# alexaiken/mpas-regent

Measured on NVIDIA B200. Metric: cell_level_updates_per_s, higher is better.
Workload: dtype f64

## Files before the change

mpas_regent_b200/csrc/kernels.cuh:

```cuda
#pragma once
#include "view.h"

#define DI __device__ __forceinline__
#ifndef LB_EDGE
#define LB_EDGE 1
#endif
#ifndef LB_CELLC
#define LB_CELLC 4
#endif
#ifndef LB_CELLC_SPLIT
#define LB_CELLC_SPLIT 5
#endif
#ifndef LB_AC
#define LB_AC 3
#endif
#ifndef KDE_PREFETCH
#define KDE_PREFETCH 1
#endif
#ifndef LB_MISC
#define LB_MISC 1
#endif
#ifndef KDE_MAXREG
#define KDE_MAXREG 56
#endif
// ... 951 lines not shown
  if (m0 && !spec && k0 > 0) s_P[k0] = ac_P(t0, s_rp0[k0 - 1], s_rt0[k0 - 1]);
  __syncthreads();
  if (inx && !spec && k0 == 0) {
    double xv = s_P[0];
#pragma unroll 4
    for (int kk = 1; kk < L; ++kk) { xv = __fma_rn(s_Q[kk], xv, s_P[kk]); s_P[kk] = xv; }
  }
  __syncthreads();
  if (!m0) return;
  const D2 ww_old = S0 ? bc(0.0) : ld2(FLD(wwAvg), ix);
  D2 rw_new, rho_new, rt_new, ww_new;
  if (!spec) {
    const D2 cofrz = ld2(FLD(cofrz), k0), rdzw = ld2(FLD(rdzw), k0);
    const D2 coftz = ld2(FLD(coftz), ix), coftz_p = above(FLD(coftz), ix, k0, L, coftz);
    const D2 rw_oldp = mk(rw_old.y, rw_oldp_y);
    rw_new = mk(s_P[k0], m1 ? s_P[k1] : 0.0);
    const D2 wa = ww_old + 0.5 * (1.0 - epssm) * rw_old;
    const D2 wb = wa + 0.5 * (1.0 + epssm) * rw_new;
    ww_new = mk(k0 > 0 ? wb.x : ww_old.x, wb.y);
    rho_new = rs - cofrz * (rw_oldp - rw_new);
    rt_new = ts - rdzw * (coftz_p * rw_oldp - coftz * rw_new);
  } else {
    const D2 rho_old = S0 ? bc(0.0) : ld2(FLD(rho_pp), ix), rt_old = S0 ? bc(0.0) : ld2(FLD(rtheta_pp), ix);
    rho_new = rho_old + dts * ld2(FLD(tend_rho), ix);
    rt_new = rt_old + dts * ld2(FLD(theta_m), ix);
    rw_new = rw_old + dts * ld2(FLD(w), ix);
    ww_new = ww_old + 0.5 * (1.0 + epssm) * rw_new;
  }
  st2m(FLD(rho_pp), ix, rho_new, m0, m1); st2m(FLD(rtheta_pp), ix, rt_new, m0, m1);
  const bool wr0 = S0 || spec || k0 > 0;
  st2m(FLD(rw_p), ix, rw_new, wr0, m1); st2m(FLD(wwAvg), ix, ww_new, wr0, m1);
}

__global__ void k_acoustic_gather(const View V, double dts) {
  PAIR_THREAD_R()
  XPF_CELL_ROWS();
  if (!m0) return;
  if (V.specZoneMaskCell[x] != 0.0) return;
  const int ME = V.maxEdges, n = V.nEdgesOnCell[x];
  const double inva = V.invAreaCell[x];
  const double* ru_p = FLD(ru_p); const double* tm = FLD(theta_m);
  D2 rs = bc(0), ts = bc(0);
#pragma unroll 2
  for (int i = 0; i < n; ++i) {
    const int e = V.edgesOnCell[x * V.MEP + i];
    const int c1 = V.c1OnCell[x * V.MEP + i], c2 = V.c2OnCell[x * V.MEP + i];
    const D2 flux = V.edgesOnCellSign[x * ME + i] * dts * V.dvOnCell[x * ME + i] * G2(ru_p, e) * inva;
    rs -= flux;
    ts -= flux * 0.5 * (G2(tm, c2) + G2(tm, c1));
  }
  st2m(V.scr_rs, ix, rs, m0, m1); st2m(V.scr_ts, ix, ts, m0, m1);
}

template <bool S0>
__global__ void k_acoustic_u(const View V, double dts, double c2, double gravity) {
  PAIR_THREAD_R()
  if (!m0) return;
  const D2 tru = ld2(FLD(tend_ru), ix);
  if (S0) {
    const D2 r = dts * tru;
    st2m(FLD(ru_p), ix, r, m0, m1); st2m(FLD(ruAvg), ix, r, m0, m1);
    return;
  }
  const int4 cv = V.ecv[x];
  const double* rpp = FLD(rtheta_pp); const double* zz = FLD(zz); const double* ex = FLD(exner); const double* rho = FLD(rho_pp);
  D2 pgrad = ((G2(rpp, cv.y) - G2(rpp, cv.x)) * V.invDcEdge[x]) / (0.5 * (G2(zz, cv.y) + G2(zz, cv.x)));
  pgrad = pgrad * (ld2(FLD(cqu), ix) * 0.5 * c2 * (G2(ex, cv.x) + G2(ex, cv.y)));
  pgrad = pgrad + 0.5 * ld2(FLD(zxu), ix) * gravity * (G2(rho, cv.x) + G2(rho, cv.y));
  const D2 r = ld2(FLD(ru_p), ix) + dts * (tru - (1.0 - V.specZoneMaskEdge[x]) * pgrad);
  st2m(FLD(ru_p), ix, r, m0, m1);
  st2m(FLD(ruAvg), ix, ld2(FLD(ruAvg), ix) + r, m0, m1);
}

template <bool S0>
__global__ void __launch_bounds__(256) k_acoustic_col(const View V, double dts, double epssm, double resm) {
  extern __shared__ double sm[];
  PAIR_THREAD_R()
  const int TS = LP + 2, CB = blockDim.y, ty = threadIdx.y;
  double* s_rs = sm + (size_t)(0 * CB + ty) * TS;
  double* s_ts = sm + (size_t)(1 * CB + ty) * TS;
  double* s_x = sm + (size_t)(2 * CB + ty) * TS;
  double* s_a = sm + (size_t)(3 * CB + ty) * TS;
// ... 209 lines not shown
    double xe = s_P[0];
#pragma unroll 4
    for (int p = 1; p < np; ++p) { xe = __fma_rn(s_Q[p], xe, s_P[p]); s_P[p] = xe; }
  }
  __syncthreads();
  if (!m0) return;
  const D2 ww_old = S0 ? bc(0.0) : ld2(SIN(AF_wwAvg), cl);
  D2 rw_new, rho_new, rt_new, ww_new;
  if (!spec) {
    const double xprev = pr > 0 ? s_P[pr - 1] : 0.0;
    const double x0 = __fma_rn(Q0, xprev, P0);
    rw_new = mk(x0, m1 ? __fma_rn(Q1, x0, P1) : 0.0);
    const D2 wa = ww_old + 0.5 * (1.0 - epssm) * rw_old;
    const D2 wb = wa + 0.5 * (1.0 + epssm) * rw_new;
    ww_new = mk(k0 > 0 ? wb.x : ww_old.x, wb.y);
    rho_new = rs - cofrz * (rw_oldp - rw_new);
    rt_new = ts - rdzw * (coftz_p * rw_oldp - coftz * rw_new);
  } else {
    rho_new = rho_old + dts * ld2(SIN(AF_tend_rho), cl);
    rt_new = rt_old + dts * ld2(SIN(AF_theta_m), cl);
    rw_new = rw_old + dts * ld2(SIN(AF_w), cl);
    ww_new = ww_old + 0.5 * (1.0 + epssm) * rw_new;
  }
  if ((ABL & 4) && rho_new.x != 1.2345e300) return;
  st2m(FLD(rho_pp), ix, rho_new, m0, m1); st2m(FLD(rtheta_pp), ix, rt_new, m0, m1);
  const bool wr0 = S0 || spec || k0 > 0;
  st2m(FLD(rw_p), ix, rw_new, wr0, m1); st2m(FLD(wwAvg), ix, ww_new, wr0, m1);
#undef SIN
}

#ifndef AL_NMOV
#define AL_NMOV 160
#endif
enum { AL_KC = 8, AL_COLS = 32, AL_NOUT = 5 };
DI void mbar_arrive(uint64_t* bar) { asm volatile("mbarrier.arrive.shared::cta.b64 _, [%0];" ::"r"(smem_u32(bar)) : "memory"); }
DI void cp_async_arrive_noinc(uint64_t* bar) { asm volatile("cp.async.mbarrier.arrive.noinc.shared::cta.b64 [%0];" ::"r"(smem_u32(bar)) : "memory"); }
DI void cp_async_16(void* dst, const void* src) { asm volatile("cp.async.cg.shared.global [%0], [%1], 16;" ::"r"(smem_u32(dst)), "l"(src) : "memory"); }
DI void cp_async_8(void* dst, const void* src) { asm volatile("cp.async.ca.shared.global [%0], [%1], 8;" ::"r"(smem_u32(dst)), "l"(src) : "memory"); }
DI int al_off(int c, int p) { return c * AL_KC + (((p ^ (c >> 1)) & 3) << 1); }
struct AcCarry { double rw_prev, rho_prev, rt_prev, zz_m, cofwt_m, rz_m; };
DI void ac_level(int k, bool spec, bool S0, double dts, double epssm, double resm, double cofrz_k, double rdzw_k, double fzm_k, double fzp_k,
                 double tend_rho_k, double theta_m_k, double w_k, double coftz_k, double coftz_p, double cofwz_k, double cofwr_k,
                 double cofwt_k, double a_k, double al_k, double zz_k, double rws_k, double rwv_k, double dsk, double rz_k, double srs_k,
                 double sts_k, double rho_old, double rt_old, double rw_old_k, double rw_old_p, double ww_old, AcCarry& c,
                 double& rho_new, double& rt_new, double& rw_new, double& ww_new) {
  ww_new = ww_old;
  if (!spec) {
    const double rs = rho_old + dts * tend_rho_k + srs_k - cofrz_k * resm * (rw_old_p - rw_old_k);
    const double ts = rt_old + dts * theta_m_k + sts_k - resm * rdzw_k * (coftz_p * rw_old_p - coftz_k * rw_old_k);
    rw_new = rw_old_k;
    if (k > 0) {
      ww_new += 0.5 * (1.0 - epssm) * rw_old_k;
      rw_new += dts * w_k - cofwz_k * ((zz_k * ts - c.zz_m * 0.0) + resm * (zz_k * rt_old - c.zz_m * c.rt_prev))
                - cofwr_k * ((rs + 0.0) + resm * (rho_old + c.rho_prev))
                + cofwt_k * (ts + resm * rt_old)
                + c.cofwt_m * (0.0 + resm * c.rt_prev);
      rw_new -= a_k * c.rw_prev;
      rw_new *= al_k;
      const double r3 = rws_k - rwv_k;
      rw_new += r3 - dts * dsk * (fzm_k * zz_k + fzp_k * c.zz_m) * (fzm_k * rz_k + fzp_k * c.rz_m) * w_k;
      const double r2 = 1.0 + dts * dsk;
      if (r2 != 1.0) rw_new /= r2;
      rw_new -= r3;
      ww_new += 0.5 * (1.0 + epssm) * rw_new;
    }
    rho_new = rs - cofrz_k * (rw_old_p - rw_new);
    rt_new = ts - rdzw_k * (coftz_p * rw_old_p - coftz_k * rw_new);
  } else {
    rho_new = rho_old + dts * tend_rho_k;
    rt_new = rt_old + dts * theta_m_k;
    rw_new = rw_old_k + dts * w_k;
    ww_new = ww_old + 0.5 * (1.0 + epssm) * rw_new;
  }
  c.rw_prev = rw_new; c.rho_prev = rho_new; c.rt_prev = rt_new; c.zz_m = zz_k; c.cofwt_m = cofwt_k; c.rz_m = rz_k;
  (void)S0;
}
template <bool S0>
__global__ void __launch_bounds__(32 + AL_NMOV, 2) k_acoustic_lane(const View V, const AcPtrs F, double dts, double epssm, double resm) {
  extern __shared__ __align__(128) unsigned char smraw[];
  constexpr int NS16 = S0 ? (int)AF_rho_pp : (int)AF_COUNT;
  constexpr int NS8 = S0 ? 1 : 2;
  constexpr int NSTR = NS16 + NS8;
  constexpr int STRIP = AL_COLS * AL_KC;
  double* in = reinterpret_cast<double*>(smraw);
  double* out = in + (size_t)2 * NSTR * STRIP;
  double* s_v = out + (size_t)2 * AL_NOUT * STRIP;
  const int L = V.L, LP = V.LP;
  uint64_t* bars = reinterpret_cast<uint64_t*>(s_v + (size_t)4 * LP);
  uint64_t* full = bars; uint64_t* empty = bars + 2; uint64_t* ofull = bars + 4; uint64_t* oempty = bars + 6;
  const int tid = threadIdx.x, warp = tid >> 5, lane = tid & 31;
  const int nch = (L + AL_KC - 1) / AL_KC;
  const int ntile = (V.xend - V.xoff + AL_COLS - 1) / AL_COLS;
  const int my_tiles = ((int)blockIdx.x < ntile) ? (ntile - 1 - (int)blockIdx.x) / (int)gridDim.x + 1 : 0;
  const int ng = my_tiles * nch;
  if (tid == 0) {
    for (int s = 0; s < 2; ++s) { mbar_init(full + s, AL_NMOV); mbar_init(empty + s, 32); mbar_init(ofull + s, 32); mbar_init(oempty + s, AL_NMOV); }
  }
  for (int i = tid; i < LP; i += blockDim.x) {
    s_v[i] = FLD(cofrz)[i]; s_v[LP + i] = FLD(rdzw)[i]; s_v[2 * LP + i] = FLD(fzm)[i]; s_v[3 * LP + i] = FLD(fzp)[i];
  }
  __syncthreads();
  if (warp == 0) {
    const int c = lane;
    int x = 0; bool on = false, spec = false;
    AcCarry cr; cr.rw_prev = cr.rho_prev = cr.rt_prev = cr.zz_m = cr.cofwt_m = cr.rz_m = 0.0;
    for (int g = 0; g < ng; ++g) {
      const int j = g % nch;
      if (j == 0) {
        x = V.xoff + ((int)blockIdx.x + (g / nch) * (int)gridDim.x) * AL_COLS + c;
        on = x < V.xend;
        spec = on ? (V.specZoneMaskCell[x] != 0.0) : false;
        cr.rw_prev = cr.rho_prev = cr.rt_prev = cr.zz_m = cr.cofwt_m = cr.rz_m = 0.0;
      }
      const int s = g & 1, u = g >> 1;
      mbar_wait(full + s, u & 1);
      if (g >= 2) mbar_wait(oempty + s, (u - 1) & 1);
      const double* __restrict__ si = in + (size_t)s * NSTR * STRIP;
      double* __restrict__ so = out + (size_t)s * AL_NOUT * STRIP;
#pragma unroll
      for (int p = 0; p < AL_KC / 2; ++p) {
        const int k0 = j * AL_KC + 2 * p;
        const int o = al_off(c, p);
#define LDP(f) (*reinterpret_cast<const D2*>(si + (size_t)(f) * STRIP + o))
        const D2 tr = LDP(AF_tend_rho), tm = LDP(AF_theta_m), w2 = LDP(AF_w), cz = LDP(AF_coftz), cwz = LDP(AF_cofwz), cwr = LDP(AF_cofwr),
                 cwt = LDP(AF_cofwt), at = LDP(AF_a_tri), al = LDP(AF_alpha_tri), zz = LDP(AF_zz), rws = LDP(AF_rw_save), rwv = LDP(AF_rw),
                 ds = LDP(AF_dss), rz = LDP(AF_rho_zz), rsh = LDP(AF_rs), tsh = LDP(AF_ts);
        const D2 czn = LDP(NS16);
        D2 rho_o = bc(0.0), rt_o = bc(0.0), rwp = bc(0.0), wwo = bc(0.0), rwpn = bc(0.0);
        if (!S0) { rho_o = LDP(AF_rho_pp); rt_o = LDP(AF_rtheta_pp); rwp = LDP(AF_rw_p); wwo = LDP(AF_wwAvg); rwpn = LDP(NS16 + 1); }
#undef LDP
        D2 rho_n = bc(0.0), rt_n = bc(0.0), rw_n = bc(0.0), ww_n = bc(0.0);
#ifdef AL_ABLATE_SWEEP
        if (false)
#else
        if (on && k0 < L)
#endif
          ac_level(k0, spec, S0, dts, epssm, resm, s_v[k0], s_v[LP + k0], s_v[2 * LP + k0], s_v[3 * LP + k0], tr.x, tm.x, w2.x, cz.x, czn.x,
                   cwz.x, cwr.x, cwt.x, at.x, al.x, zz.x, rws.x, rwv.x, ds.x, rz.x, rsh.x, tsh.x, rho_o.x, rt_o.x, rwp.x, rwpn.x, wwo.x, cr,
                   rho_n.x, rt_n.x, rw_n.x, ww_n.x);
#ifdef AL_ABLATE_SWEEP
        if (false)
#else
        if (on && k0 + 1 < L)
#endif
          ac_level(k0 + 1, spec, S0, dts, epssm, resm, s_v[k0 + 1], s_v[LP + k0 + 1], s_v[2 * LP + k0 + 1], s_v[3 * LP + k0 + 1], tr.y, tm.y, w2.y,
                   cz.y, czn.y, cwz.y, cwr.y, cwt.y, at.y, al.y, zz.y, rws.y, rwv.y, ds.y, rz.y, rsh.y, tsh.y, rho_o.y, rt_o.y, rwp.y, rwpn.y,
                   wwo.y, cr, rho_n.y, rt_n.y, rw_n.y, ww_n.y);
        *reinterpret_cast<D2*>(so + (size_t)0 * STRIP + o) = rho_n;
        *reinterpret_cast<D2*>(so + (size_t)1 * STRIP + o) = rt_n;
        *reinterpret_cast<D2*>(so + (size_t)2 * STRIP + o) = rw_n;
        *reinterpret_cast<D2*>(so + (size_t)3 * STRIP + o) = ww_n;
        *reinterpret_cast<D2*>(so + (size_t)4 * STRIP + o) = rt_o;
      }
      mbar_arrive(empty + s);
      mbar_arrive(ofull + s);
      if (S0 && on && j == nch - 1) { FLD(wwAvg)[(size_t)x * LP + L] = 0; FLD(rw_p)[(size_t)x * LP + L] = 0; }
    }
  } else {
    const int m = tid - 32;
    double* const dst_f[AL_NOUT] = {FLD(rho_pp), FLD(rtheta_pp), FLD(rw_p), FLD(wwAvg), FLD(rtheta_pp_old)};
    const int xl = V.xend - 1;
    for (int g = 0; g <= ng; ++g) {
      if (g < ng) {
        const int s = g & 1, u = g >> 1;
        if (g >= 2) mbar_wait(empty + s, (u - 1) & 1);
        double* si = in + (size_t)s * NSTR * STRIP;
        const int kb = (g % nch) * AL_KC;
        const int x0 = V.xoff + ((int)blockIdx.x + (g / nch) * (int)gridDim.x) * AL_COLS;
        for (int it = m; it < NS16 * (AL_COLS * 4); it += AL_NMOV) {
          const int f = it >> 7, cp = it & 127, c = cp >> 2, p = cp & 3;
          const int xc = min(x0 + c, xl);
          cp_async_16(si + (size_t)f * STRIP + al_off(c, p), F.p[f] + (size_t)xc * LP + kb + 2 * p);
        }
        for (int it = m; it < NS8 * (AL_COLS * 8); it += AL_NMOV) {
          const int f = it >> 8, ck = it & 255, c = ck >> 3, kk = ck & 7;
          const int xc = min(x0 + c, xl);
          const double* src = (f == 0 ? F.p[AF_coftz] : F.p[AF_rw_p]) + (size_t)xc * LP + kb + kk + 1;
          cp_async_8(si + (size_t)(NS16 + f) * STRIP + al_off(c, kk >> 1) + (kk & 1), src);
        }
        cp_async_arrive_noinc(full + s);
      }
      if (g >= 1) {
        const int gg = g - 1, s = gg & 1, u = gg >> 1;
        mbar_wait(ofull + s, u & 1);
        const double* so = out + (size_t)s * AL_NOUT * STRIP;
        const int kb = (gg % nch) * AL_KC;
        const int x0 = V.xoff + ((int)blockIdx.x + (gg / nch) * (int)gridDim.x) * AL_COLS;
        for (int it = m; it < AL_NOUT * (AL_COLS * 4); it += AL_NMOV) {
          const int f = it >> 7, cp = it & 127, c = cp >> 2, p = cp & 3;
          const int x = x0 + c, k0 = kb + 2 * p;
          const D2 v = *reinterpret_cast<const D2*>(so + (size_t)f * STRIP + al_off(c, p));
          if (x < V.xend && k0 < L) st2m(dst_f[f], (size_t)x * LP + k0, v, true, k0 + 1 < L);
        }
        mbar_arrive(oempty + s);
      }
    }
  }
}

__global__ void k_acoustic_flux(const View V, double dts, int small_step) {
  const int k = threadIdx.x;
  const int x = blockIdx.x * blockDim.y + threadIdx.y;
  if (x >= V.nCells) return;
  const int LP = V.LP, L = V.L;
  const size_t ix = (size_t)x * LP + k;
  if (k == L && small_step == 0) { FLD(wwAvg)[ix] = 0; FLD(rw_p)[ix] = 0; }
  if (k >= L) return;
  FLD(rtheta_pp_old)[ix] = (small_step == 0) ? 0.0 : FLD(rtheta_pp)[ix];
  if (V.specZoneMaskCell[x] != 0.0) return;
  const int ME = V.maxEdges, n = V.nEdgesOnCell[x];
  const double* ru_p = FLD(ru_p); const double* tm = FLD(theta_m);
  const double inva = V.invAreaCell[x];
  double rs = 0, ts = 0;
  for (int i = 0; i < n; ++i) {
    const int e = V.edgesOnCell[x * V.MEP + i];
    const int c1 = V.c1OnCell[x * V.MEP + i], c2 = V.c2OnCell[x * V.MEP + i];
    const double flux = V.edgesOnCellSign[x * ME + i] * dts * V.dvOnCell[x * ME + i] * G1(ru_p, e, k) * inva;
    rs -= flux;
    ts -= flux * 0.5 * (G1(tm, c2, k) + G1(tm, c1, k));
  }
  V.scr_rs[ix] = rs; V.scr_ts[ix] = ts;
}
__global__ void k_acoustic_column(const View V, double dts, int small_step, double epssm, double resm) {
  const int c = blockIdx.x * blockDim.x + threadIdx.x;
  if (c >= V.nCells) return;
  const int L = V.L, LP = V.LP;
  const size_t b = (size_t)c * LP;
  const bool S0 = small_step == 0;
// ... 453 lines not shown
```

mpas_regent_b200/csrc/mpas_b200.cu:

```cuda
#include <cuda_runtime.h>
#include <dlfcn.h>

#include <algorithm>
#include <cmath>
#include <cstdio>
#include <cstddef>
#include <cstdlib>
#include <cstring>
#include <map>
#include <mutex>
#include <numeric>
#include <string>
#include <vector>

#include "kernels.cuh"
#ifdef MPASB200_LAB
#include "kernels_tiles.cuh"
#endif
#include "kernels_init.cuh"
#include "kernels_jw.cuh"
#ifdef MPASB200_LAB
#include "kernels_staged.cuh"
#include "kernels_lab.cuh"
#endif
// ... 384 lines not shown
Range range_of(const mpasb200_t* h, int ent, int n) {
  if (!h->rangeSet[ent]) return Range{0, n, n, true};
  const int b = std::min(h->rangeB[ent], n), e = std::min(h->rangeE[ent], n);
  return Range{b, e, std::max(0, e - b), b == 0 && e == n};
}
View ranged(const mpasb200_t* h, const Range& r) { View v = h->V; v.xoff = r.b; v.xend = r.e; return v; }
int t_smlstep(mpasb200_t* h) { LAUNCH(k_smlstep, h->nCells, 0, h->V, h->c.nRelaxZone); return post_launch(h); }
int t_acoustic(mpasb200_t* h, double dts, int small_step) {
  const double epssm = h->c.config_epssm;
  const double resm = (1.0 - epssm) / (1.0 + epssm);
  const Range rc_ = range_of(h, MPASB200_CELL, h->nCells), re_ = range_of(h, MPASB200_EDGE, h->nEdges);
  const View Vc = ranged(h, rc_), Ve = ranged(h, re_);
  const size_t sm_gather = staged_bytes(h, 12, 0);
  if (h->c.physics_mode == MPASB200_PHYSICS_CORRECTED) {
    const double rcv = h->c.rgas / (h->c.cp - h->c.rgas), c2 = h->c.cp * rcv;
    if (small_step == 0) LAUNCH(k_acoustic_u<true>, re_.n, 0, Ve, dts, c2, h->c.gravity);
    else LAUNCH(k_acoustic_u<false>, re_.n, 0, Ve, dts, c2, h->c.gravity);
    if (staged_on(h, GS_AC_GATHER, sm_gather)) LAUNCH_STAGED(k_acoustic_gather_s<6>, rc_.n, sm_gather, Vc, dts);
    else LAUNCH(k_acoustic_gather, rc_.n, 0, Vc, dts);
    if (small_step == 0) LAUNCH(k_acoustic_col<true>, rc_.n, tile_bytes(h, 6), Vc, dts, epssm, resm);
    else LAUNCH(k_acoustic_col<false>, rc_.n, tile_bytes(h, 6), Vc, dts, epssm, resm);
    return post_launch(h);
  }
  {
    const size_t smem_lane = ((size_t)2 * (AF_COUNT + 2) * AL_COLS * AL_KC + (size_t)2 * AL_NOUT * AL_COLS * AL_KC + (size_t)4 * h->LP) * sizeof(double) + 64;
    if (!h->c.acoustic_exact && h->c.acoustic_tma == 3 && smem_lane <= (size_t)h->max_smem_optin) {
      if (rc_.n == 0) return 0;
      const View& V = Vc;
      AcPtrs F;
#define AF(n) F.p[AF_##n] = V.f[MPASB200_F_##n]
      AF(tend_rho); AF(theta_m); AF(w); AF(coftz); AF(cofwz); AF(cofwr); AF(cofwt); AF(a_tri); AF(alpha_tri); AF(zz); AF(rw_save); AF(rw);
      AF(dss); AF(rho_zz); AF(rho_pp); AF(rtheta_pp); AF(rw_p); AF(wwAvg);
#undef AF
      F.p[AF_rs] = V.scr_rs; F.p[AF_ts] = V.scr_ts;
      LAUNCH(k_acoustic_gather, rc_.n, 0, Vc, dts);
      static bool attr_ = false;
      if (!attr_) {
        cudaFuncSetAttribute(k_acoustic_lane<true>, cudaFuncAttributeMaxDynamicSharedMemorySize, h->max_smem_optin);
        cudaFuncSetAttribute(k_acoustic_lane<false>, cudaFuncAttributeMaxDynamicSharedMemorySize, h->max_smem_optin);
        attr_ = true;
      }
      const size_t smem0 = ((size_t)2 * ((int)AF_rho_pp + 1) * AL_COLS * AL_KC + (size_t)2 * AL_NOUT * AL_COLS * AL_KC + (size_t)4 * h->LP) * sizeof(double) + 64;
      const int tiles = (rc_.n + AL_COLS - 1) / AL_COLS;
      const dim3 grid(std::min(tiles, 2 * h->num_sms)), block(32 + AL_NMOV);
      {
        KTimer kt_(h, small_step == 0 ? "k_acoustic_lane<true>" : "k_acoustic_lane<false>");
        if (small_step == 0) k_acoustic_lane<true><<<grid, block, smem0, h->stream>>>(V, F, dts, epssm, resm);
        else k_acoustic_lane<false><<<grid, block, smem_lane, h->stream>>>(V, F, dts, epssm, resm);
      }
      h->launches++;
      return post_launch(h);
    }
  }
  const bool tma_fits = ((size_t)AF_COUNT * h->LP + (size_t)4 * (h->LP + 2)) * sizeof(double) + 16 <= 48 * 1024 && h->LP / 2 <= 128;
  if (!h->c.acoustic_exact && h->c.acoustic_tma && h->nCells > 0 && tma_fits) {
    if (rc_.n == 0) return 0;
    const View& V = Vc;
    AcPtrs F;
#define AF(n) F.p[AF_##n] = V.f[MPASB200_F_##n]
    AF(tend_rho); AF(theta_m); AF(w); AF(coftz); AF(cofwz); AF(cofwr); AF(cofwt); AF(a_tri); AF(alpha_tri); AF(zz); AF(rw_save); AF(rw);
    AF(dss); AF(rho_zz); AF(rho_pp); AF(rtheta_pp); AF(rw_p); AF(wwAvg);
#undef AF
    F.p[AF_rs] = V.scr_rs; F.p[AF_ts] = V.scr_ts;
    const int split = h->c.acoustic_tma == 2;
    if (split) {
      if (staged_on(h, GS_AC_GATHER, sm_gather)) LAUNCH_STAGED(k_acoustic_gather_s<6>, rc_.n, sm_gather, Vc, dts);
      else LAUNCH(k_acoustic_gather, rc_.n, 0, Vc, dts);
    }
    const int T = h->LP / 2, NF = small_step == 0 ? (int)AF_rho_pp : (int)AF_COUNT;
    int C = 4;
    auto smem_for = [&](int c) { return ((size_t)NF * c * h->LP + (size_t)4 * c * (h->LP + 2)) * sizeof(double) + 16; };
    while (C > 1 && (smem_for(C) > 48 * 1024 || C * T > 128)) C /= 2;
    const size_t smem = smem_for(C);
    dim3 block(T, C), grid((rc_.n + C - 1) / C);
// ... 354 lines not shown
  c->config_horiz_mixing = MPASB200_MIX_2D_SMAGORINSKY;
  c->nRelaxZone = 5; c->number_of_sub_steps = 2; c->config_dynamics_split_steps = 1;
  c->index_policy = MPASB200_INDEX_CORRECTED; c->rkarg_policy = MPASB200_RKARG_SUBSTEP_TRUNC;
  c->sfc_renumber = 1; c->device = -1; c->use_graph = 0; c->acoustic_exact = 0; c->acoustic_tma = 3;
  c->physics_mode = MPASB200_PHYSICS_LITERAL;
  c->gather_stage = 0;
  c->config_scalar_advection = 0; c->config_coef_3rd_order = 0.25;
  c->edge_tiles = 0; c->kernel_forms = 0; c->reserved0 = 0;
}

const char* mpasb200_last_error(const mpasb200_t* h) { return h ? h->err.c_str() : g_create_error.c_str(); }

int mpasb200_create(const MpasDims* dims, const MpasConfig* cfg, mpasb200_t** out) {
  if (!dims || !cfg || !out) return fail(nullptr, MPASB200_EINVAL, "null argument");
  if (dims->nCells < 0 || dims->nEdges < 0 || dims->nVertices < 0 || dims->nVertLevels < 3)
    return fail(nullptr, MPASB200_EINVAL, "bad dimensions (nVertLevels must be >= 3)");
  if (dims->maxEdges < 1 || dims->maxEdges > 16 || dims->nAdvCells < 1 || dims->vertexDegree != 3)
    return fail(nullptr, MPASB200_EINVAL, "unsupported maxEdges / nAdvCells / vertexDegree");
  int ndev = 0;
  cudaError_t e = cudaGetDeviceCount(&ndev);
  if (e != cudaSuccess || ndev == 0)
    return fail(nullptr, MPASB200_ENODEVICE, std::string("no CUDA device (") + cudaGetErrorString(e) + "); libmpas_b200 has no host path");
  mpasb200_t* h = new mpasb200();
  h->d = *dims; h->c = *cfg;
  if (cfg->device >= 0) h->device = cfg->device; else cudaGetDevice(&h->device);
  if ((e = cudaSetDevice(h->device)) != cudaSuccess) { g_create_error = std::string("cudaSetDevice: ") + cudaGetErrorString(e); delete h; return MPASB200_ECUDA; }
  h->nCells = dims->nCells; h->nEdges = dims->nEdges; h->nVertices = dims->nVertices;
  h->L = dims->nVertLevels; h->L1 = h->L + 1; h->LP = (h->L1 + 3) / 4 * 4;
  { const int T = h->LP / 2; int g = T, b = 32; while (b) { int t = g % b; g = b; b = t; } h->CPB = 32 / g; while (h->CPB * T < 128) h->CPB *= 2;
    while (h->CPB * T > 256 && h->CPB > 1) h->CPB /= 2; }
  if (h->LP / 2 * h->CPB > 256) { g_create_error = "nVertLevels too large for one block per column group"; delete h; return MPASB200_EINVAL; }
  cudaDeviceGetAttribute(&h->num_sms, cudaDevAttrMultiProcessorCount, h->device);
  cudaDeviceGetAttribute(&h->max_smem_optin, cudaDevAttrMaxSharedMemoryPerBlockOptin, h->device);
  cudaStreamCreateWithFlags(&h->own_stream, cudaStreamNonBlocking);
  h->stream = h->own_stream;
  cudaEventCreate(&h->ev0); cudaEventCreate(&h->ev1);
  View& V = h->V;
  std::memset(&V, 0, sizeof(V));
  V.nCells = h->nCells; V.nEdges = h->nEdges; V.nVertices = h->nVertices; V.L = h->L; V.LP = h->LP;
  V.xoff = 0; V.xend = 0;
  V.maxEdges = dims->maxEdges; V.maxEdges2 = dims->maxEdges2; V.vertexDegree = dims->vertexDegree; V.nAdv = dims->nAdvCells;
  V.cellSlot = (size_t)(h->nCells + 1) * h->LP;
  size_t total = 0;
  std::vector<size_t> off(MPASB200_F_COUNT);
  for (int id = 0; id < MPASB200_F_COUNT; ++id) {
    size_t n = (kFields[id].entity == MPASB200_VERTICAL) ? (size_t)h->LP
                                                         : (size_t)(entity_count(h, kFields[id].entity) + 1) * h->LP * kFields[id].slots;
    n = (n + 15) / 16 * 16;
    off[id] = total; total += n;
  }
  const size_t scr = ((size_t)(h->nCells + 1) * h->LP + 15) / 16 * 16;
  double* arena = nullptr;
  const size_t scr_e = ((size_t)(h->nEdges + 1) * h->LP + 15) / 16 * 16;
  int rc = dev_alloc(h, &arena, total + 2 * scr + scr_e + (size_t)16 * h->LP);
  if (rc) { g_create_error = h->err; mpasb200_destroy(h); return rc; }
  for (int id = 0; id < MPASB200_F_COUNT; ++id) V.f[id] = arena + off[id];
  V.scr_rs = arena + total; V.scr_ts = arena + total + scr; V.scr_flux = arena + total + 2 * scr;
  if (cudaStreamSynchronize(h->stream) != cudaSuccess) { g_create_error = "arena memset failed"; mpasb200_destroy(h); return MPASB200_ECUDA; }
  *out = h;
  return 0;
}

int mpasb200_destroy(mpasb200_t* h) {
  if (!h) return 0;
  cudaSetDevice(h->device);
  cudaDeviceSynchronize();
// ... 1108 lines not shown
```

mpas_regent_b200/traffic.py:

```python
from __future__ import annotations

from typing import Dict, List, Tuple

from ._abi import CELL, EDGE, FIELD_ENTITY, FIELD_SLOTS, VERTEX

MULT = {CELL: 1, EDGE: 3, VERTEX: 2}

USED_SLOTS = 6

K: Dict[str, Tuple[List[str], List[str]]] = {
    "k_setup_cell": (["rw", "rtheta_p", "rho_p", "w", "theta_m", "rho_zz"],
                     ["rw_save", "rtheta_p_save", "rho_p_save", "w_2", "theta_m_2", "rho_zz_2", "rho_zz_old_split"]),
    "k_setup_edge": (["ru", "u"], ["ru_save", "u_2"]),
    "k_moist": ([], ["qtot", "cqw"]),
    "k_vert_imp": (["zz", "cqw", "exner", "theta_m", "qtot", "rho_base", "rtheta_base", "rtheta_p", "exner_base", "gamma_tri"],
                   ["cofwr", "cofwz", "coftz", "cofwt", "a_tri", "b_tri", "c_tri", "alpha_tri", "gamma_tri"]),
    "k_diag_vertex": (["u"], ["vorticity", "pv_vertex"]),
    "k_diag_cell": (["u"], ["divergence", "ke"]),
    "k_diag_edge<false>": (["h", "u", "pv_vertex"], ["h_edge", "ke_edge", "pv_edge"]),
    "k_diag_edge<true>": (["h", "u", "pv_vertex"], ["h_edge", "ke_edge", "pv_edge", "v"]),
    "k_diag_ke_vertex": (["ke_edge"], ["ke_vertex"]),
    "k_diag_ke_holl": (["ke", "ke_vertex"], ["ke"]),
    "k_dt_cell0<true>": (["u", "v", "ru", "rw", "tend_rho_physics", "qtot", "rho_base", "rho_p_save"],
                         ["kdiff", "h_divergence", "tend_rho", "dpdz"]),
# ... 33 lines not shown
    "k_acoustic<true>": (["ru_p", "theta_m", "tend_rho", "w", "coftz", "cofwz", "cofwr", "cofwt", "a_tri", "alpha_tri", "zz",
                          "rw_save", "rw", "dss", "rho_zz"], ["rtheta_pp_old", "rho_pp", "rtheta_pp", "rw_p", "wwAvg"]),
    "k_acoustic<false>": (["ru_p", "theta_m", "tend_rho", "w", "coftz", "cofwz", "cofwr", "cofwt", "a_tri", "alpha_tri", "zz",
                           "rw_save", "rw", "dss", "rho_zz", "rho_pp", "rtheta_pp", "rw_p", "wwAvg"],
                          ["rtheta_pp_old", "rho_pp", "rtheta_pp", "rw_p", "wwAvg"]),
    "k_acoustic_gather": (["ru_p", "theta_m"], ["scr", "scr"]),
    "k_acoustic_u<true>": (["tend_ru"], ["ru_p", "ruAvg"]),
    "k_acoustic_u<false>": (["tend_ru", "rtheta_pp", "zz", "exner", "rho_pp", "cqu", "zxu", "ru_p", "ruAvg"], ["ru_p", "ruAvg"]),
    "k_acoustic_col<true>": (["scr", "scr", "theta_m", "tend_rho", "w", "coftz", "cofwz", "cofwr", "cofwt", "a_tri", "alpha_tri", "gamma_tri",
                              "zz", "rw_save", "rw", "dss", "rho_zz"], ["rtheta_pp_old", "rho_pp", "rtheta_pp", "rw_p", "wwAvg"]),
    "k_acoustic_col<false>": (["scr", "scr", "theta_m", "tend_rho", "w", "coftz", "cofwz", "cofwr", "cofwt", "a_tri", "alpha_tri", "gamma_tri",
                               "zz", "rw_save", "rw", "dss", "rho_zz", "rho_pp", "rtheta_pp", "rw_p", "wwAvg"],
                              ["rtheta_pp_old", "rho_pp", "rtheta_pp", "rw_p", "wwAvg"]),
    "k_divdamp": (["rtheta_pp", "rtheta_pp_old", "theta_m", "ru_p"], ["ru_p"]),
    "k_rec_cell1": (["rho_p_save", "rho_pp", "rho_base", "wwAvg", "rw_save", "rw_p", "zz", "rtheta_base", "rtheta_p_save",
                     "rtheta_pp"], ["rho_p", "rho_zz", "wwAvg", "rw", "w", "rtheta_p", "theta_m"]),
    "k_rec_edge": (["ruAvg", "ru_save", "ru_p", "rho_zz"], ["ruAvg", "ru", "u"]),
    "k_rec_cell2": (["w", "ru", "zb_cell", "zb3_cell", "rho_zz"], ["w"]),
    "k_finish_cell": (["wwAvg", "rho_zz_old_split"], ["wwAvg_split", "wwAvg", "rho_zz"]),
    "k_finish_edge": (["ruAvg"], ["ruAvg_split", "ruAvg"]),
    "k_icd_cell1": (["rho_zz", "zz"], ["rho_zz"]),
    "k_icd_edge": (["u", "rho_zz"], ["ru"]),
    "k_icd_cell2": (["w", "rho_zz", "zz", "ru", "zb_cell", "zb3_cell", "rho_base", "theta_base", "theta_m"],
                    ["rw", "rho_p", "rtheta_base", "rtheta_p", "exner", "exner_base", "pressure_p", "pressure_base"]),
    "k_reconstruct": (["u"], ["uReconstructX", "uReconstructY", "uReconstructZ", "uReconstructZonal", "uReconstructMeridional"]),
    "k_zb_cell": (["zb", "zb3"], ["zb_cell", "zb3_cell"]),
    "k_damping_coefs": (["zgrid"], ["dss"]),
    "k_jw_rw": (["zz", "ru", "rho_zz", "zb"], ["rw", "w"]),
    "k_setup_scalars": (["scalars"], ["scalars_old"]),
    "k_scalar_flux<NS>": (["ruAvg", "scalars"], ["scr_e"] * 8),
    "k_scalar_update<NS>": (["ruAvg", "scalars", "scalars_old", "wwAvg", "rho_zz", "rho_zz_old_split"] + ["scr_e"] * 8, ["scalars"]),
}
K["k_dt_edge_tile"] = K["k_dt_edge"]
K["k_acoustic_lane<true>"] = K["k_acoustic_tma<true>"]
K["k_acoustic_lane<false>"] = K["k_acoustic_tma<false>"]
FULL_SLOTS = {"scalars": 8, "scalars_old": 8, "zb": 2, "zb3": 2}


def canon(kernel: str) -> str:
    import re
    m = re.match(r"(k_\w+?)_s<\d+>$", kernel)
    return m.group(1) if m else kernel


def lookup(kernel: str):
    k = canon(kernel)
    return k if k in K else None


def _u(name: str) -> float:
    if name == "scr":
        return 1.0
    if name == "scr_e":
        return 3.0
    s = FIELD_SLOTS[name]
    return MULT[FIELD_ENTITY[name]] * (FULL_SLOTS.get(name, USED_SLOTS) if s > 1 else 1)


def units(kernel: str, scratch: bool = True) -> float:
    r, w = K[canon(kernel)]
    return sum(_u(n) for n in r + w if scratch or not n.startswith("scr"))


def step_launches(canonical: bool = True, corrected_physics: bool = False) -> List[str]:
    seq = ["k_setup_cell", "k_setup_edge", "k_moist", "k_vert_imp"]
    for stage in range(3):
        if stage == 1:
            seq.append("k_vert_imp")
        if stage == 0 and canonical:
            seq += ["k_dt_cell0<true>", "k_dt_edge_delsq", "k_dt_vertex_delsq", "k_dt_cell_delsq", "k_dt_edge_euler", "k_dt_edge",
                    "k_dt_cellA", "k_dt_cellB", "k_dt_theta_flux", "k_dt_cellC<true>"]
        else:
            seq += ["k_dt_cell0<false>", "k_dt_edge", "k_dt_theta_flux", "k_dt_cellC<false>"]
        seq.append("k_smlstep")
        for ss in range((1 if stage < 2 else 2) + 1):
            t = "<true>" if ss == 0 else "<false>"
            if corrected_physics:
                seq += ["k_acoustic_u" + t, "k_acoustic_gather", "k_acoustic_col" + t, "k_divdamp"]
            else:
                seq += ["k_acoustic_gather", "k_acoustic_lane" + t, "k_divdamp"]
        if corrected_physics:
            seq += ["k_rec_pad", "k_rec_cell1", "k_rec_edge", "k_rec_cell2"]
        seq += ["k_diag_vertex", "k_diag_cell", "k_diag_edge<true>" if stage == 2 else "k_diag_edge<false>"]
    seq += ["k_finish_cell", "k_finish_edge"]
    return seq


def step_units(canonical: bool = True, scratch: bool = True, corrected_physics: bool = False) -> float:
    return sum(units(k, scratch) for k in step_launches(canonical, corrected_physics) if k != "k_rec_pad")


SURVEY_TASK_UNITS = {
    "rk_integration_setup": 25, "compute_moist_coefficients": 2, "compute_vert_imp_coefs": 19,
    "compute_dyn_tend:rk0": 96, "compute_dyn_tend:rk>0": 53, "set_smlstep_pert_variables": 18,
    "advance_acoustic_step:s0": 22, "advance_acoustic_step": 26, "divergence_damping_3d": 9,
    "compute_solve_diagnostics": 24, "compute_solve_diagnostics:v": 27, "rk_dynamics_substep_finish": 14,
}
SURVEY_STEP_UNITS_CANONICAL = 643
SURVEY_STEP_UNITS_LITERAL = 600

TASK_KERNELS = {
    "rk_integration_setup": ["k_setup_cell", "k_setup_edge"],
    "compute_moist_coefficients": ["k_moist"],
    "compute_vert_imp_coefs": ["k_vert_imp"],
    "compute_dyn_tend:rk0": ["k_dt_cell0<true>", "k_dt_edge_delsq", "k_dt_vertex_delsq", "k_dt_cell_delsq", "k_dt_edge_euler", "k_dt_edge",
                             "k_dt_cellA", "k_dt_cellB", "k_dt_theta_flux", "k_dt_cellC<true>"],
    "compute_dyn_tend:rk>0": ["k_dt_cell0<false>", "k_dt_edge", "k_dt_theta_flux", "k_dt_cellC<false>"],
    "set_smlstep_pert_variables": ["k_smlstep"],
    "advance_acoustic_step:s0": ["k_acoustic_gather", "k_acoustic_lane<true>"],
    "advance_acoustic_step": ["k_acoustic_gather", "k_acoustic_lane<false>"],
    "advance_acoustic_step:s0:affine": ["k_acoustic_gather", "k_acoustic_tma<true>"],
    "advance_acoustic_step:affine": ["k_acoustic_gather", "k_acoustic_tma<false>"],
    "advance_scalars": ["k_scalar_flux<NS>", "k_scalar_update<NS>"],
    "advance_acoustic_step:s0:fused": ["k_acoustic<true>"],
    "advance_acoustic_step:fused": ["k_acoustic<false>"],
    "advance_acoustic_step:s0:exact": ["k_acoustic_flux:s0", "k_acoustic_column:s0"],
    "advance_acoustic_step:exact": ["k_acoustic_flux", "k_acoustic_column"],
    "advance_acoustic_step:s0:corrected_physics": ["k_acoustic_u<true>", "k_acoustic_gather", "k_acoustic_col<true>"],
    "advance_acoustic_step:corrected_physics": ["k_acoustic_u<false>", "k_acoustic_gather", "k_acoustic_col<false>"],
    "recover_large_step_variables": ["k_rec_cell1", "k_rec_edge", "k_rec_cell2"],
    "divergence_damping_3d": ["k_divdamp"],
    "compute_solve_diagnostics": ["k_diag_vertex", "k_diag_cell", "k_diag_edge<false>"],
    "compute_solve_diagnostics:v": ["k_diag_vertex", "k_diag_cell", "k_diag_edge<true>"],
    "rk_dynamics_substep_finish": ["k_finish_cell", "k_finish_edge"],
}


def task_units(task: str, scratch: bool = False) -> float:
    return sum(units(k, scratch) for k in TASK_KERNELS[task])
```

Measured before the change: 642.2 million.

## Fuse acoustic horizontal flux gather into lane kernel producer warps

Removes the separate k_acoustic_gather launch and computes the per-cell rs/ts horizontal flux sums inside k_acoustic_lane's mover warps. The sums are written straight into the shared staging strips, and the cp.async copies of the scratch fields are skipped. Gather loads for the next chunk are issued before the current one is consumed, so their latency overlaps the pipeline. The full barrier now expects twice as many arrivals. The shared-memory attribute setup also moves from the step path into create. The cost is more register pressure in the producer warps and extra global gather traffic inside the lane kernel.

```diff
diff --git a/mpas_regent_b200/csrc/kernels.cuh b/mpas_regent_b200/csrc/kernels.cuh
--- a/mpas_regent_b200/csrc/kernels.cuh
+++ b/mpas_regent_b200/csrc/kernels.cuh
@@ -1007,6 +1007,12 @@
   st2m(FLD(rw_p), ix, rw_new, wr0, m1); st2m(FLD(wwAvg), ix, ww_new, wr0, m1);
 }
 
+DI void ac_flux_slot(double sign, double dts, double dv, D2 ru, double inva, D2 tm1, D2 tm2, D2& rs, D2& ts) {
+  const D2 flux = sign * dts * dv * ru * inva;
+  rs -= flux;
+  ts -= flux * 0.5 * (tm2 + tm1);
+}
+
 __global__ void k_acoustic_gather(const View V, double dts) {
   PAIR_THREAD_R()
   XPF_CELL_ROWS();
@@ -1020,9 +1026,7 @@
   for (int i = 0; i < n; ++i) {
     const int e = V.edgesOnCell[x * V.MEP + i];
     const int c1 = V.c1OnCell[x * V.MEP + i], c2 = V.c2OnCell[x * V.MEP + i];
-    const D2 flux = V.edgesOnCellSign[x * ME + i] * dts * V.dvOnCell[x * ME + i] * G2(ru_p, e) * inva;
-    rs -= flux;
-    ts -= flux * 0.5 * (G2(tm, c2) + G2(tm, c1));
+    ac_flux_slot(V.edgesOnCellSign[x * ME + i], dts, V.dvOnCell[x * ME + i], G2(ru_p, e), inva, G2(tm, c1), G2(tm, c2), rs, ts);
   }
   st2m(V.scr_rs, ix, rs, m0, m1); st2m(V.scr_ts, ix, ts, m0, m1);
 }
@@ -1298,12 +1302,47 @@
 #ifndef AL_NMOV
 #define AL_NMOV 160
 #endif
+#ifndef AL_GORDER
+#define AL_GORDER 2
+#endif
 enum { AL_KC = 8, AL_COLS = 32, AL_NOUT = 5 };
 DI void mbar_arrive(uint64_t* bar) { asm volatile("mbarrier.arrive.shared::cta.b64 _, [%0];" ::"r"(smem_u32(bar)) : "memory"); }
 DI void cp_async_arrive_noinc(uint64_t* bar) { asm volatile("cp.async.mbarrier.arrive.noinc.shared::cta.b64 [%0];" ::"r"(smem_u32(bar)) : "memory"); }
 DI void cp_async_16(void* dst, const void* src) { asm volatile("cp.async.cg.shared.global [%0], [%1], 16;" ::"r"(smem_u32(dst)), "l"(src) : "memory"); }
 DI void cp_async_8(void* dst, const void* src) { asm volatile("cp.async.ca.shared.global [%0], [%1], 8;" ::"r"(smem_u32(dst)), "l"(src) : "memory"); }
 DI int al_off(int c, int p) { return c * AL_KC + (((p ^ (c >> 1)) & 3) << 1); }
+enum { AL_GS = 6 };
+struct AlGather { D2 ru[AL_GS], ta[AL_GS], tb[AL_GS]; int x, k0, n; double inva; };
+DI void al_gather_issue(const View& V, int x, int k0, AlGather& G) {
+  const int LP = V.LP, ME = V.maxEdges;
+  const int* eo = V.edgesOnCell + (size_t)x * V.MEP; const int* o1 = V.c1OnCell + (size_t)x * V.MEP; const int* o2 = V.c2OnCell + (size_t)x * V.MEP;
+  const double* ru_p = FLD(ru_p); const double* tm = FLD(theta_m);
+  const bool spec = V.specZoneMaskCell[x] != 0.0;
+  const int nr = V.nEdgesOnCell[x];
+  G.x = x; G.k0 = k0; G.n = spec ? 0 : nr; G.inva = V.invAreaCell[x];
+  int e[AL_GS], c1[AL_GS], c2[AL_GS];
+#pragma unroll
+  for (int i = 0; i < AL_GS; ++i) {
+    if (i < ME) { e[i] = eo[i]; c1[i] = o1[i]; c2[i] = o2[i]; }
+    else e[i] = c1[i] = c2[i] = 0;
+  }
+#pragma unroll
+  for (int i = 0; i < AL_GS; ++i) {
+    if (i < G.n) { G.ru[i] = G2(ru_p, e[i]); G.ta[i] = G2(tm, c1[i]); G.tb[i] = G2(tm, c2[i]); }
+    else G.ru[i] = G.ta[i] = G.tb[i] = bc(0.0);
+  }
+}
+DI void al_gather_sum(const View& V, const AlGather& G, double dts, D2& rs, D2& ts) {
+  const int LP = V.LP, ME = V.maxEdges, x = G.x, k0 = G.k0, n = G.n;
+  const double* sg = V.edgesOnCellSign + (size_t)x * ME; const double* dv = V.dvOnCell + (size_t)x * ME;
+  rs = bc(0), ts = bc(0);
+#pragma unroll
+  for (int i = 0; i < AL_GS; ++i)
+    if (i < n) ac_flux_slot(sg[i], dts, dv[i], G.ru[i], G.inva, G.ta[i], G.tb[i], rs, ts);
+  const int* eo = V.edgesOnCell + (size_t)x * V.MEP; const int* o1 = V.c1OnCell + (size_t)x * V.MEP; const int* o2 = V.c2OnCell + (size_t)x * V.MEP;
+  const double* ru_p = FLD(ru_p); const double* tm = FLD(theta_m);
+  for (int i = AL_GS; i < n; ++i) ac_flux_slot(sg[i], dts, dv[i], G2(ru_p, eo[i]), G.inva, G2(tm, o1[i]), G2(tm, o2[i]), rs, ts);
+}
 struct AcCarry { double rw_prev, rho_prev, rt_prev, zz_m, cofwt_m, rz_m; };
 DI void ac_level(int k, bool spec, bool S0, double dts, double epssm, double resm, double cofrz_k, double rdzw_k, double fzm_k, double fzp_k,
                  double tend_rho_k, double theta_m_k, double w_k, double coftz_k, double coftz_p, double cofwz_k, double cofwr_k,
@@ -1360,7 +1399,7 @@
   const int my_tiles = ((int)blockIdx.x < ntile) ? (ntile - 1 - (int)blockIdx.x) / (int)gridDim.x + 1 : 0;
   const int ng = my_tiles * nch;
   if (tid == 0) {
-    for (int s = 0; s < 2; ++s) { mbar_init(full + s, AL_NMOV); mbar_init(empty + s, 32); mbar_init(ofull + s, 32); mbar_init(oempty + s, AL_NMOV); }
+    for (int s = 0; s < 2; ++s) { mbar_init(full + s, 2 * AL_NMOV); mbar_init(empty + s, 32); mbar_init(ofull + s, 32); mbar_init(oempty + s, AL_NMOV); }
   }
   for (int i = tid; i < LP; i += blockDim.x) {
     s_v[i] = FLD(cofrz)[i]; s_v[LP + i] = FLD(rdzw)[i]; s_v[2 * LP + i] = FLD(fzm)[i]; s_v[3 * LP + i] = FLD(fzp)[i];
@@ -1426,6 +1465,24 @@
     const int m = tid - 32;
     double* const dst_f[AL_NOUT] = {FLD(rho_pp), FLD(rtheta_pp), FLD(rw_p), FLD(wwAvg), FLD(rtheta_pp_old)};
     const int xl = V.xend - 1;
+    AlGather G;
+    bool gon = false;
+    auto gather_issue = [&](int g) {
+      const int x = V.xoff + ((int)blockIdx.x + (g / nch) * (int)gridDim.x) * AL_COLS + (m >> 2), k0 = (g % nch) * AL_KC + 2 * (m & 3);
+      gon = m < AL_COLS * 4 && x < V.xend && k0 < L;
+      if (gon) al_gather_issue(V, x, k0, G);
+    };
+    auto gather_done = [&](int g) {
+      if (gon) {
+        double* si = in + (size_t)(g & 1) * NSTR * STRIP;
+        const int o = al_off(m >> 2, m & 3);
+        D2 rs, ts;
+        al_gather_sum(V, G, dts, rs, ts);
+        *reinterpret_cast<D2*>(si + (size_t)AF_rs * STRIP + o) = rs;
+        *reinterpret_cast<D2*>(si + (size_t)AF_ts * STRIP + o) = ts;
+      }
+      mbar_arrive(full + (g & 1));
+    };
     for (int g = 0; g <= ng; ++g) {
       if (g < ng) {
         const int s = g & 1, u = g >> 1;
@@ -1433,8 +1490,8 @@
         double* si = in + (size_t)s * NSTR * STRIP;
         const int kb = (g % nch) * AL_KC;
         const int x0 = V.xoff + ((int)blockIdx.x + (g / nch) * (int)gridDim.x) * AL_COLS;
-        for (int it = m; it < NS16 * (AL_COLS * 4); it += AL_NMOV) {
-          const int f = it >> 7, cp = it & 127, c = cp >> 2, p = cp & 3;
+        for (int it = m; it < (NS16 - 2) * (AL_COLS * 4); it += AL_NMOV) {
+          const int fi = it >> 7, f = fi < (int)AF_rs ? fi : fi + 2, cp = it & 127, c = cp >> 2, p = cp & 3;
           const int xc = min(x0 + c, xl);
           cp_async_16(si + (size_t)f * STRIP + al_off(c, p), F.p[f] + (size_t)xc * LP + kb + 2 * p);
         }
@@ -1445,6 +1502,16 @@
           cp_async_8(si + (size_t)(NS16 + f) * STRIP + al_off(c, kk >> 1) + (kk & 1), src);
         }
         cp_async_arrive_noinc(full + s);
+#if AL_GORDER == 2
+        if (g == 0) gather_issue(0);
+        gather_done(g);
+        if (g + 1 < ng) gather_issue(g + 1);
+#else
+        gather_issue(g);
+#if AL_GORDER == 0
+        gather_done(g);
+#endif
+#endif
       }
       if (g >= 1) {
         const int gg = g - 1, s = gg & 1, u = gg >> 1;
@@ -1460,6 +1527,9 @@
         }
         mbar_arrive(oempty + s);
       }
+#if AL_GORDER == 1
+      if (g < ng) gather_done(g);
+#endif
     }
   }
 }
diff --git a/mpas_regent_b200/csrc/mpas_b200.cu b/mpas_regent_b200/csrc/mpas_b200.cu
--- a/mpas_regent_b200/csrc/mpas_b200.cu
+++ b/mpas_regent_b200/csrc/mpas_b200.cu
@@ -440,14 +440,7 @@
       AF(tend_rho); AF(theta_m); AF(w); AF(coftz); AF(cofwz); AF(cofwr); AF(cofwt); AF(a_tri); AF(alpha_tri); AF(zz); AF(rw_save); AF(rw);
       AF(dss); AF(rho_zz); AF(rho_pp); AF(rtheta_pp); AF(rw_p); AF(wwAvg);
 #undef AF
-      F.p[AF_rs] = V.scr_rs; F.p[AF_ts] = V.scr_ts;
-      LAUNCH(k_acoustic_gather, rc_.n, 0, Vc, dts);
-      static bool attr_ = false;
-      if (!attr_) {
-        cudaFuncSetAttribute(k_acoustic_lane<true>, cudaFuncAttributeMaxDynamicSharedMemorySize, h->max_smem_optin);
-        cudaFuncSetAttribute(k_acoustic_lane<false>, cudaFuncAttributeMaxDynamicSharedMemorySize, h->max_smem_optin);
-        attr_ = true;
-      }
+      F.p[AF_rs] = F.p[AF_ts] = nullptr;
       const size_t smem0 = ((size_t)2 * ((int)AF_rho_pp + 1) * AL_COLS * AL_KC + (size_t)2 * AL_NOUT * AL_COLS * AL_KC + (size_t)4 * h->LP) * sizeof(double) + 64;
       const int tiles = (rc_.n + AL_COLS - 1) / AL_COLS;
       const dim3 grid(std::min(tiles, 2 * h->num_sms)), block(32 + AL_NMOV);
@@ -868,6 +861,10 @@
   if (h->LP / 2 * h->CPB > 256) { g_create_error = "nVertLevels too large for one block per column group"; delete h; return MPASB200_EINVAL; }
   cudaDeviceGetAttribute(&h->num_sms, cudaDevAttrMultiProcessorCount, h->device);
   cudaDeviceGetAttribute(&h->max_smem_optin, cudaDevAttrMaxSharedMemoryPerBlockOptin, h->device);
+  for (const void* k : {(const void*)k_acoustic_lane<true>, (const void*)k_acoustic_lane<false>})
+    if ((e = cudaFuncSetAttribute(k, cudaFuncAttributeMaxDynamicSharedMemorySize, h->max_smem_optin)) != cudaSuccess) {
+      g_create_error = std::string("cudaFuncSetAttribute(k_acoustic_lane): ") + cudaGetErrorString(e); delete h; return MPASB200_ECUDA;
+    }
   cudaStreamCreateWithFlags(&h->own_stream, cudaStreamNonBlocking);
   h->stream = h->own_stream;
   cudaEventCreate(&h->ev0); cudaEventCreate(&h->ev1);
diff --git a/mpas_regent_b200/traffic.py b/mpas_regent_b200/traffic.py
--- a/mpas_regent_b200/traffic.py
+++ b/mpas_regent_b200/traffic.py
@@ -89,8 +89,8 @@
     "k_scalar_update<NS>": (["ruAvg", "scalars", "scalars_old", "wwAvg", "rho_zz", "rho_zz_old_split"] + ["scr_e"] * 8, ["scalars"]),
 }
 K["k_dt_edge_tile"] = K["k_dt_edge"]
-K["k_acoustic_lane<true>"] = K["k_acoustic_tma<true>"]
-K["k_acoustic_lane<false>"] = K["k_acoustic_tma<false>"]
+K["k_acoustic_lane<true>"] = K["k_acoustic<true>"]
+K["k_acoustic_lane<false>"] = K["k_acoustic<false>"]
 FULL_SLOTS = {"scalars": 8, "scalars_old": 8, "zb": 2, "zb3": 2}
 
 
@@ -143,8 +143,13 @@
     return seq
 
 
+def library_step_launches(canonical: bool = True, corrected_physics: bool = False) -> List[str]:
+    seq = step_launches(canonical, corrected_physics)
+    return seq if corrected_physics else [k for k in seq if k != "k_acoustic_gather"]
+
+
 def step_units(canonical: bool = True, scratch: bool = True, corrected_physics: bool = False) -> float:
-    return sum(units(k, scratch) for k in step_launches(canonical, corrected_physics) if k != "k_rec_pad")
+    return sum(units(k, scratch) for k in library_step_launches(canonical, corrected_physics) if k != "k_rec_pad")
 
 
 SURVEY_TASK_UNITS = {
@@ -164,8 +169,8 @@
                              "k_dt_cellA", "k_dt_cellB", "k_dt_theta_flux", "k_dt_cellC<true>"],
     "compute_dyn_tend:rk>0": ["k_dt_cell0<false>", "k_dt_edge", "k_dt_theta_flux", "k_dt_cellC<false>"],
     "set_smlstep_pert_variables": ["k_smlstep"],
-    "advance_acoustic_step:s0": ["k_acoustic_gather", "k_acoustic_lane<true>"],
-    "advance_acoustic_step": ["k_acoustic_gather", "k_acoustic_lane<false>"],
+    "advance_acoustic_step:s0": ["k_acoustic_lane<true>"],
+    "advance_acoustic_step": ["k_acoustic_lane<false>"],
     "advance_acoustic_step:s0:affine": ["k_acoustic_gather", "k_acoustic_tma<true>"],
     "advance_acoustic_step:affine": ["k_acoustic_gather", "k_acoustic_tma<false>"],
     "advance_scalars": ["k_scalar_flux<NS>", "k_scalar_update<NS>"],
```

Result: slower. 621.0 million (median of 6 runs) (-3.3%).
